# nvpro-samples/vk_gltf_renderer

Hardware: AMD Instinct MI355X
Metric: Msamples/s (and ms/frame @ fixed spp) 1080p & 4K, 1/2/4/8 MI355X (higher is better)
Workload: dtype f32

## Files before the change

### vk_gltf_renderer_amd/csrc/device/mi_pt_api.hip

```cpp
#include <hip/hip_runtime.h>

#include <algorithm>
#include <chrono>
#include <cstdlib>
#include <cmath>
#include <cstdio>
#include <cstring>
#include <memory>
#include <string>
#include <vector>

#include "mi_pt.h"
#include "bvh_refit.h"
#include "material_patch.h"
#include "pt_build.h"
#include "pt_bvh.h"
#include "pt_deform.h"
#include "pt_kernels.h"

namespace {

thread_local std::string g_lastError;

int fail(int code, const std::string& msg)
// ... 17 lines not shown
  size_t count = 0;
  hipError_t alloc(size_t n)
  {
    release();
    count = n;
    if(n == 0)
      return hipSuccess;
    return hipMalloc(reinterpret_cast<void**>(&ptr), n * sizeof(T));
  }
  hipError_t upload(const T* src, size_t n)
  {
    hipError_t e = alloc(n);
    if(e != hipSuccess || n == 0)
      return e;
    return hipMemcpy(ptr, src, n * sizeof(T), hipMemcpyHostToDevice);
  }
  void release()
  {
    if(ptr)
      (void)hipFree(ptr);
    ptr   = nullptr;
    count = 0;
  }
  ~DevBuf() { release(); }
};

enum TimedKernel { TK_GENERATE, TK_TRACE, TK_SORT, TK_SHADE, TK_SHADOW, TK_ACCUM, TK_PRIMARY, TK_SHADE_FIRST, TK_COUNT };

}

struct RunSwitches
{
  int    packetInterval = 1;
  int    sortMode       = 2;
  bool   noPacket       = false;
  bool   stateBySlot    = false;
  bool   traceSpans     = false;
  int    overlapUpTo    = 32;
  int    overlapMinTris = 200000;
  bool   noPlanes       = false;
  bool   noOpaqueTris   = false;
  bool   noQuads        = false;
  bool   shadowFarFirst = true;
  int    reinsert       = 16;
  int    reinsertUpdate = 0;
  int    reinsertRounds = 4;
  float  splitFactor    = 4.0f;
  int    splitMaxDepth  = 8;
  float  splitMinShare  = 0.1f;
  bool   collapseGreedy = false;
  bool   collapseBad    = false;
  bool   hostCollapse   = false;
  bool   coreTex        = true;
  int    maxItersDiag   = 0;
  int    failBuildAt    = 0;
  bool   candPoolSet    = false;
  size_t candPool       = 0;
  void   read()
  {
    auto flag = [](const char* n) { const char* e = getenv(n); return e != nullptr; };
    auto num  = [](const char* n, int d) { const char* e = getenv(n); return e ? atoi(e) : d; };
    packetInterval = num("MI_PT_PACKET_INTERVAL", 1);
    sortMode       = num("MI_PT_SORT", 2);
    noPacket       = flag("MI_PT_NO_PACKET");
    stateBySlot    = flag("MI_PT_STATE_BY_SLOT");
    traceSpans     = flag("MI_PT_TRACE_SPANS");
    overlapUpTo    = num("MI_PT_OVERLAP", 32);
    overlapMinTris = num("MI_PT_OVERLAP_MIN_TRIS", 200000);
    noPlanes       = flag("MI_PT_DIAG_NO_PLANES");
    noOpaqueTris   = flag("MI_PT_DIAG_NO_OPAQUE_TRIS");
    noQuads        = flag("MI_PT_DIAG_NO_QUADS");
    shadowFarFirst = num("MI_PT_SHADOW_FAR_FIRST", 1) != 0;
    reinsert       = std::max(0, num("MI_PT_REINSERT", 16));
    reinsertUpdate = std::max(0, num("MI_PT_REINSERT_UPDATE", 0));
    reinsertRounds = std::max(1, num("MI_PT_REINSERT_ROUNDS", 4));
    if(const char* e = getenv("MI_PT_SPLIT"))
      splitFactor = std::max(0.0f, float(atof(e)));
    if(const char* e = getenv("MI_PT_SPLIT_MIN_SHARE"))
      splitMinShare = std::max(0.0f, float(atof(e)));
    splitMaxDepth  = std::min(std::max(0, num("MI_PT_SPLIT_DEPTH", 8)), 10);
    if(const char* e = getenv("MI_PT_COLLAPSE"))
    {
      collapseGreedy = strcmp(e, "greedy") == 0;
      collapseBad    = !collapseGreedy && strcmp(e, "sah") != 0;
    }
    hostCollapse   = flag("MI_PT_HOST_COLLAPSE");
    maxItersDiag   = num("MI_PT_DIAG_MAX_ITERS", 0);
    coreTex        = num("MI_PT_CORE_TEX", 1) != 0;
    failBuildAt    = num("MI_PT_DIAG_FAIL_BUILD", 0);
    if(const char* e = getenv("MI_PT_DIAG_CAND_POOL"))
    {
      candPoolSet = true;
      candPool    = size_t(strtoull(e, nullptr, 10));
    }
  }
};

struct MiPt
{
  int device = 0;
  int numCUs = 256;
  RunSwitches sw;
  int accelBuilds = 0;
  int               frameQueueDepth = 1;
  int               pendingFrames   = 0;
  MiPathtraceParams pendingFirst{};
  void*             pendingStream   = nullptr;
  DevBuf<MiGltfShadeMaterial> materials;
  DevBuf<MiGltfTextureInfo>   texInfos;
  DevBuf<pt::DevTexRef>       texRefs;
  DevBuf<pt::DevCoreTex>      coreTex;
  DevBuf<MiGltfRenderNode>    nodes;
  DevBuf<pt::DevPrim>         prims;
  DevBuf<MiGltfLight>         lights;
  DevBuf<pt::DevTexture>      textures;
  DevBuf<uchar4>              texels;
  DevBuf<uint4>               texQuads;
  DevBuf<uint8_t>             geometry;
  DevBuf<uint8_t>             instFlags;
  DevBuf<float>               srgbLut;
  DevBuf<float4>              envPixels;
  DevBuf<MiEnvAccel>          envAccel;
  DevBuf<pt::DevAlphaTri>     alphaTris;
  DevBuf<pt::DevShadeTri>     shadeTris;
  float4*                     bvhNodes  = nullptr;
  uint4*                      bvh8Nodes = nullptr;
  DevBuf<float>               bvh8Planes;
  pt::DevTri*                 bvhTris   = nullptr;
  bool                        wide      = true;
  pt::DevScene                scene{};
  bool                        hasAlpha = false, hasAlphaTest = false, hasVolumeScatter = false, simpleMaterials = true, hasTransmissive = false;
  static constexpr int        FC_RING = 32;
  DevBuf<pt::DevScene>        sceneDev;
  bool                        sceneDevDirty = true;
  DevBuf<pt::FrameConsts>     fcRing;
  DevBuf<pt::SkyPrecomp>      skyPre;
  MiSkyPhysicalParameters     skyPreFor{};
  bool                        skyPreValid = false;
  pt::FrameConsts*            fcHost = nullptr;
  hipEvent_t                  fcDone[FC_RING] = {};
  unsigned                    fcCursor = 0;
// ... 1845 lines not shown
  }
  c.fc.skyPre    = pt->skyPre.ptr;
  c.fc.pc        = *params;
  c.fc.width     = pt->width;
  c.fc.height    = pt->height;
  c.fc.tileSize  = pt->tileSize;
  c.fc.tileShift = 0;
  while((1 << c.fc.tileShift) < pt->tileSize)
    ++c.fc.tileShift;
  c.fc.numSlots  = pt->numSlots;
  c.fc.numFrames = numFrames;
  pt::divideMagic(uint32_t(std::max(numFrames, 2)), c.fc.framesMagic, c.fc.framesShift);
  c.fc.slotLayout = numFrames % 64 == 0 ? 1 : 0;
  c.fc.stateInQueue = (!pt->sw.stateBySlot && !(pt->frameInfo.flags & MI_SCENE_INFINITE_PLANE_SHADOW_CATCHER)) ? 1 : 0;
  const bool guides = (params->flags & MI_PT_USE_OPTIX_DENOISER) != 0;
  if(int rc = ensureOptionalPathArrays(pt, c.fc.stateInQueue == 0, params->numSamples > 1, guides, (pt->frameInfo.flags & MI_SCENE_INFINITE_PLANE_SHADOW_CATCHER) != 0))
    return rc;
  c.paths        = pt->paths;
  {
    const bool stateBySlot = c.fc.stateInQueue == 0, multiSample = params->numSamples > 1;
    if(!(stateBySlot || multiSample))
      c.paths.misc = nullptr;
    if(!stateBySlot)
      c.paths.throughput = nullptr;
    if(!multiSample)
      c.paths.pixelSum = nullptr;
  }
  pt->accumFrames   = float(params->totalSamples) / float(params->numSamples) + float(numFrames);
  if(guides && (params->totalSamples == 0 || pt->momentFrames == pt->accumFrames - float(numFrames)))
    pt->momentFrames = pt->accumFrames;
  else if(!guides || params->totalSamples == 0)
    pt->momentFrames = 0.0f;
  if(!guides)
  {
    c.paths.guideAlbedo = nullptr;
    c.paths.guideNormal = nullptr;
  }
  c.queues           = pt->queues;
  if(!(pt->frameInfo.flags & MI_SCENE_INFINITE_PLANE_SHADOW_CATCHER))
    c.queues.shadow.aux2 = nullptr;
  c.ownedTiles       = pt->ownedTiles.ptr;
  c.stats            = pt->stats.ptr;
  c.stream           = stream;
  c.persistentBlocks = unsigned(pt->numCUs) * 8u;
  c.hasAlpha         = pt->hasAlpha;
  c.hasAlphaClosest  = c.hasAlpha && pt->hasAlphaTest;
  c.visualization    = pt->frameInfo.visualization > MI_VIZ_RENDERED && pt->frameInfo.visualization < MI_VIZ_COUNT;
  if(pt->frameInfo.visualization == MI_VIZ_OPACITY_MICROMAP)
    c.hasAlphaClosest = false;
  c.hasTransmissive  = pt->hasTransmissive;
  c.simpleMaterials  = pt->simpleMaterials;
  c.wide             = pt->wide;
  c.collectCounters  = pt->collectCounters;
  {
    c.sortMode = pt->sw.sortMode;
  }
  if(pt->sceneDevDirty)
  {
    HIP_TRY(hipDeviceSynchronize());
    HIP_TRY(pt->sceneDev.upload(&pt->scene, 1));
    pt->sceneDevDirty = false;
  }
  if(!pt->fcHost)
  {
    HIP_TRY(hipHostMalloc(reinterpret_cast<void**>(&pt->fcHost), sizeof(pt::FrameConsts) * MiPt::FC_RING, hipHostMallocDefault));
    HIP_TRY(pt->fcRing.alloc(MiPt::FC_RING));
    for(hipEvent_t& e : pt->fcDone)
      HIP_TRY(hipEventCreateWithFlags(&e, hipEventDisableTiming));
  }
  const unsigned fcSlot = pt->fcCursor++ % unsigned(MiPt::FC_RING);
  if(pt->fcCursor > unsigned(MiPt::FC_RING))
    HIP_TRY(hipEventSynchronize(pt->fcDone[fcSlot]));
  pt->fcHost[fcSlot] = c.fc;
  HIP_TRY(hipMemcpyAsync(pt->fcRing.ptr + fcSlot, pt->fcHost + fcSlot, sizeof(pt::FrameConsts), hipMemcpyHostToDevice, stream));
  c.sceneDev = pt->sceneDev.ptr;
  c.fcDev    = pt->fcRing.ptr + fcSlot;

  auto timedOn = [&](hipStream_t on, int kind, auto&& launch) {
    if(pt->timingEnabled)
    {
      hipEvent_t a = getEvent(pt, pt->evCursor), b = getEvent(pt, pt->evCursor);
      (void)hipEventRecord(a, on);
      launch();
      (void)hipEventRecord(b, on);
      pt->pendingSpans.push_back({kind, a, b});
    }
    else
      launch();
  };
  auto timed = [&](int kind, auto&& launch) { timedOn(stream, kind, launch); };
  hipEvent_t frameA = nullptr, frameB = nullptr;
  if(pt->timingEnabled)
  {
    frameA = getEvent(pt, pt->evCursor);
    frameB = getEvent(pt, pt->evCursor);
    (void)hipEventRecord(frameA, stream);
  }
  int iterations = 0, traceLaunches = 0, shadeLaunches = 0, shadowLaunches = 0;
  const bool usePacket = !pt->sw.noPacket;
  const bool debugSpans = pt->sw.traceSpans;
  bool overlap = pt->sw.overlapUpTo > 0 && ((numFrames <= pt->sw.overlapUpTo && pt->scene.numTris >= pt->sw.overlapMinTris) || pt->hasVolumeScatter)
                 && c.fc.stateInQueue != 0 && !debugSpans;
  if(overlap && !pt->sideStream)
    overlap = hipStreamCreateWithFlags(&pt->sideStream, hipStreamNonBlocking) == hipSuccess && hipEventCreateWithFlags(&pt->evShaded, hipEventDisableTiming) == hipSuccess
              && hipEventCreateWithFlags(&pt->evShadowed, hipEventDisableTiming) == hipSuccess;
  pt::LaunchCtx cSide = c;
// ... 618 lines not shown
```

### vk_gltf_renderer_amd/csrc/device/pt_kernels.h

```cpp
#pragma once
#include <hip/hip_runtime.h>

#include "pt_scene.h"
#include "pt_temporal.h"

namespace pt {

struct LaunchCtx
{
  DevScene        scene;
  FrameConsts     fc;
  const DevScene*    sceneDev;
  const FrameConsts* fcDev;
  PathSoA         paths;
  Queues          queues;
  const uint32_t* ownedTiles;
  StatCounters*   stats;
  hipStream_t     stream;
  unsigned        persistentBlocks;
  bool            hasAlpha;
  bool            hasAlphaClosest;
  bool            hasTransmissive;
  bool            simpleMaterials;
  bool            wide;
  bool            collectCounters;
  int             sortMode;
  bool            visualization;
};

void launchBuildShadeRecords(const DevScene& scene, uint32_t numTris, DevShadeTri* out, hipStream_t s);
void launchBuildAlphaRecords(const DevScene& scene, uint32_t numTris, DevAlphaTri* out, hipStream_t s);
void launchPatchMaterials(const DevScene& scene, const uint8_t* instFlags, const uint8_t* dirty, DevTri* tris, DevAlphaTri* alphaTris, DevShadeTri* shadeTris,
                          uint32_t numTris, hipStream_t s);
void dumpTraceProfile();
void launchBvh8Planes(const uint4* nodes, uint32_t numNodes, float* planes, hipStream_t s);
void launchTextureQuads(const uchar4* texels, uint4* quads, uint32_t offset, int width, int height, int wrapS, int wrapT, hipStream_t s);
void launchResetCounters(const Queues& Q, hipStream_t s);
void launchSkyPrecomp(const MiSkyPhysicalParameters& sky, SkyPrecomp* out, hipStream_t stream);
void launchGenerate(const LaunchCtx& c, int sampleIndex);
void launchTraceClosest(const LaunchCtx& c, int cur);
void launchTracePrimary(const LaunchCtx& c, int sampleIndex);
void launchShade(const LaunchCtx& c, int cur, bool first);
void launchTraceShadow(const LaunchCtx& c, int nxt);
void launchFlushSurvivors(const LaunchCtx& c, int cur);
void launchFinishSample(const LaunchCtx& c, int sampleIndex, float4* accum, float* depth, float4* albedo, float4* normal);
void launchSelection(const LaunchCtx& c, uint32_t* selection);

void launchAtrous(const float4* in, float4* out, const float4* albedo, const float4* normal, int width, int height, int step, float sigmaColor,
                  float sigmaNormal, float sigmaAlbedo, hipStream_t s);

const float4* launchSvgf(const float4* color, const float4* albedo, const float4* normal, const float* depth, float4* bufA, float4* bufB, int width, int height,
                         int iterations, float frames, float sigmaLuminance, float sigmaNormal, float sigmaDepth, hipStream_t s);

const float4* launchSvgfFilter(float4* in, float4* other, const float4* color, const float4* albedo, const float4* normal, const float* depth, int width,
                               int height, int iterations, float sigmaLuminance, float sigmaNormal, float sigmaDepth, hipStream_t s);

void launchMotionVectors(const float4* firstHit, const uint4* firstHitTri, const VertexMotionPrim* vmPrims, int numPrims, const uint32_t* ownedTiles,
                         uint32_t numSlots, int tileShift, int width, int height, const MiGltfRenderNode* nodes, float* prevObjectToWorld, int numNodes,
                         const float* viewProj, const float* prevMVP, float4* motion, hipStream_t s);
void launchSnapshotTransforms(const MiGltfRenderNode* nodes, float* prevObjectToWorld, int numNodes, hipStream_t s);
void launchSnapshotPositions(const VertexMotionPrim* vmPrims, const uint32_t* ids, uint32_t numIds, uint32_t maxVertexCount, hipStream_t s);
void launchSvgfReproject(const float4* color, const float4* albedo, const float4* normal, const float* depth, const float4* motion, const TemporalHistory& in,
                         const TemporalHistory& out, float4* illum, int width, int height, const TemporalConsts& tc, bool haveHistory, hipStream_t s);

void launchTonemap(const float4* in, uint32_t* outRgba8, int width, int height, const MiTonemapperData& tm, uint32_t* histogram, float* autoState,
                   float dtSeconds, hipStream_t s);

}
```

### vk_gltf_renderer_amd/csrc/device/pt_kernels.hip

```cpp
#include <hip/hip_runtime.h>
#include <hip/hip_fp16.h>

#ifndef MI_PT_EXACT_FP
#define PT_FAST_SHADING_MATH 1
#endif
#include "pt_kernels.h"
#include "pt_shading.h"
#include "pt_bvh.h"
#include "pt_bvh8.h"
#include "pt_packet.h"
#include "pt_feed.h"
#include "pt_visualize.h"

namespace pt {

namespace {

constexpr int TRACE_BLOCK = 1024;
#ifndef NODE_CACHE_EXTRA
#define NODE_CACHE_EXTRA 0
#endif
constexpr int NODE_CACHE  = 712 + NODE_CACHE_EXTRA;
constexpr int NODE_CACHE_ALPHA = 504 + NODE_CACHE_EXTRA;
constexpr int SEL_BLOCK   = 256;
// ... 1298 lines not shown
        const uint32_t child = groupPopChild(G, octinv);
        if(G.bits >> 8)
          st2.push(G);
        uint32_t tBase, tMask;
        bvh8Visit(sc, r, bestT, octinv, child, G, tBase, tMask, nullptr, 0u);
        while(leafPending(tMask))
        {
          const int k = int(leafPop(tMask, 0u));
          testTri(int(tBase) + k);
        }
      }
    }
    else
    {
      LaneStack st;
      int       stackOverflow[BVH_STACK_PRIV];
      st.lds = s_stack; st.tid = int(threadIdx.x); st.stride = SEL_BLOCK; st.sp = 0; st.priv = stackOverflow;
      bvhWalk(sc, r, bestT, st, [&](int triIndex, float) -> float {
        testTri(triIndex);
        return bestT;
      });
    }
  }
  selection[size_t(py) * size_t(fc.width) + size_t(px)] = (bestRnode != 0xffffffffu) ? bestRnode + 1u : 0u;
}

template <bool COUNT, bool SIMPLE, bool FIRST>
__global__ void __launch_bounds__(SHADE_BLOCK, SIMPLE ? SHADE_SIMPLE_WAVES : 1) k_shade(const DevScene* __restrict__ scp, const FrameConsts* __restrict__ fcp, PathSoA P, Queues Q, int cur, int sortMode, StatCounters* stats)
{
  constexpr bool VIZ = false;
#include "pt_shade_body.h"
}
template <bool SIMPLE, bool FIRST>
__global__ void __launch_bounds__(SHADE_BLOCK, SIMPLE ? SHADE_SIMPLE_WAVES : 1) k_shade_viz(const DevScene* __restrict__ scp, const FrameConsts* __restrict__ fcp, PathSoA P, Queues Q, int cur, int sortMode, StatCounters* stats)
{
  constexpr bool COUNT = false, VIZ = true;
#include "pt_shade_body.h"
}

template <int MODE>
struct ShadowCfg
{
  static constexpr int BLOCK = MODE == 2 ? 256 : TRACE_BLOCK;
  static constexpr int CACHE = MODE == 2 ? 320 : (MODE == 1 ? NODE_CACHE_ALPHA : (MODE == 3 ? NODE_CACHE_ALPHA - 104 : NODE_CACHE));
};

PT_DEV void shadowDeposit(const PathSoA& P, const Queues& Q, int nxt, uint32_t slot, uint32_t qpos, bool catcherRay, f3 contrib, f3 total, bool occ,
                          float catcherDarken)
{
  if(!catcherRay)
  {
    if(!occ)
    {
      float4* const target = (slot & SHADOW_TARGET_QUEUE) ? &Q.active[nxt].rad[slot & ~SHADOW_TARGET_QUEUE] : &P.radiance[slot];
      float4        rad    = *target;
      rad.x += contrib.x * total.x;
      rad.y += contrib.y * total.y;
      rad.z += contrib.z * total.z;
      *target = rad;
    }
    return;
  }
  const float4 a2  = Q.shadow.aux2[qpos];
  const f3     sf  = occ ? mk3(0.0f) : total;
  float4       rad = P.radiance[slot];
  if(sf.x == 1.0f && sf.y == 1.0f && sf.z == 1.0f)
  {
    rad.x += a2.x; rad.y += a2.y; rad.z += a2.z;
    const uint32_t posNext = __float_as_uint(a2.w);
    if(posNext != 0xffffffffu)
      Q.active[nxt].slot[posNext] = QUEUE_DEAD;
  }
  else
  {
    f3 r3 = mk3(rad.x, rad.y, rad.z);
    r3 += contrib * sf;
    r3 -= contrib * (mk3(1.0f) - sf) * catcherDarken;
    rad.x = r3.x; rad.y = r3.y; rad.z = r3.z;
  }
  P.radiance[slot] = rad;
}

template <bool WIDE, int MODE, bool COUNT>
__global__ void __launch_bounds__(ShadowCfg<MODE>::BLOCK, TRACE_MIN_WAVES) k_trace_shadow(DevScene sc, const DevScene* __restrict__ scp, PathSoA P, Queues Q, int nxt, float catcherDarken, StatCounters* stats, int overflowOnly)
{
  constexpr int  SBLOCK    = ShadowCfg<MODE>::BLOCK;
  constexpr bool HAS_ALPHA = MODE >= 1, HAS_TRANS = MODE == 2, REC = MODE == 3;
  constexpr bool DEFER = MODE == 1 || MODE == 3;
  static_assert(!REC || WIDE, "the recording walk exists for the 8-wide BVH only");
  __shared__ int      s_stack[BVH_STACK_LDS * SBLOCK];
  __shared__ uint32_t s_prefix[NSUB + 1];
  __shared__ uint4    s_nodes[WIDE ? ShadowCfg<MODE>::CACHE * 5 : 1];
  __shared__ uint32_t s_items[(WIDE && !HAS_TRANS) ? SBLOCK : 1];
  __shared__ uint4    s_alpha[(WIDE && DEFER) ? SBLOCK : 1];
  __shared__ uint32_t s_head[REC ? SBLOCK : 1], s_ovf[REC ? SBLOCK : 1];
  __shared__ uint8_t  s_octLut[(WIDE && MI_PT_OCT_LUT) ? OCT_LUT_BYTES : 1];
  queuePrefix(&Q.counters[(nxt ? QC_PAIR1 : QC_PAIR0) + 1], s_prefix);
  const RayQueue in = Q.shadow;
  const bool     subset = MODE == 2 && overflowOnly != 0;
  uint32_t* const heads = &Q.counters[subset ? QC_HEADS_OVERFLOW : QC_HEADS_SHADOW];
  WaveFeed feed;
  feedInit(feed, subset ? Q.counters[QC_OVERFLOW] : s_prefix[NSUB]);
  if(!feedBlockHasWork(feed))
    return;
  if(WIDE && MI_PT_OCT_LUT)
    fillOctLut(s_octLut);
  const uint32_t cachedNodes = WIDE ? fillNodeCache(sc, s_nodes, uint32_t(ShadowCfg<MODE>::CACHE)) : 0u;
  LaneStack  st;
  LaneStack2 st2;
  int        stackOverflow[WIDE ? 2 * BVH8_STACK_PRIV : BVH_STACK_PRIV];
  st.lds = s_stack;  st.tid = int(threadIdx.x);  st.stride = SBLOCK;  st.sp = 0;  st.priv = stackOverflow;
  st2.lds = s_stack; st2.tid = int(threadIdx.x); st2.stride = SBLOCK; st2.sp = 0;
  st2.privBase = reinterpret_cast<uint32_t*>(stackOverflow); st2.privBits = reinterpret_cast<uint32_t*>(stackOverflow) + (WIDE ? BVH8_STACK_PRIV : 0);
  bool      active = false;
  uint32_t  slot   = 0;
  RaySetup  r{};
  int       node = BVH_EMPTY;
  NodeGroup G{0, 0};
  uint32_t  octinv = 0;
  float     tMax  = 0.0f;
  int       phase = 0;
  unsigned  nTrans = 0;
  bool      occluded = false;
  uint32_t  seed0 = 0;
  f3        contrib = mk3(0.0f);
  float    bT = 0.0f, bU = 0.0f, bV = 0.0f, lastT = -1.0f, prevHitT = 0.0f;
  uint32_t bRnode = 0, bPrim = 0, lastRnode = 0, lastPrim = 0;
  int      bTri = 0;
  bool     found = false, haveLast = false, isInside = false;
  f3       total = mk3(1.0f);
  unsigned nodes = 0, tris = 0, rays = 0;
  bool     pValid = false;
  uint32_t pSlot = QUEUE_DEAD, pQPos = 0, qpos = 0;
  float4   pO = make_float4(0, 0, 0, 0), pD = make_float4(0, 0, 0, 0), pC = make_float4(0, 0, 0, 0);
  bool     catcherRay = false;
  uint32_t pBase = 0, pMask = 0, qBase = 0, qMask = 0;
  uint32_t aCount   = 0;
  bool     aPending = false;
  bool     toOverflow = false;
#ifdef TRACE_PROFILE
  unsigned long long sp[16] = {0, 0, 0, 0, 0, 0, 0, 0, 0, 0, 0, 0, 0, 0, 0, 0};
  const unsigned long long spStart = PROF_T();
#define SPROF_ADD(i, t0) sp[i] += PROF_T() - (t0)
#define SPROF_CNT(i, n) sp[i] += (unsigned long long)(n)
#else
#define SPROF_ADD(i, t0) (void)(t0)
#define SPROF_CNT(i, n) (void)0
#endif
  uint4*   waveAlpha = s_alpha + ((WIDE && DEFER) ? (threadIdx.x & ~63u) : 0u);
  CandRec  rec{Q.candPool, Q.candNext, &Q.counters[QC_CAND_POOL], Q.candCap, s_head + (REC ? (threadIdx.x & ~63u) : 0u), s_ovf + (REC ? (threadIdx.x & ~63u) : 0u), 0u, 0u};
  (void)rec;

  auto deposit = [&](bool occ) { shadowDeposit(P, Q, nxt, slot, qpos, catcherRay, contrib, total, occ, catcherDarken); };

  constexpr unsigned SHADOW_CANDS = 8;
  float    cT[HAS_TRANS ? SHADOW_CANDS : 1], cU[HAS_TRANS ? SHADOW_CANDS : 1], cV[HAS_TRANS ? SHADOW_CANDS : 1];
  uint32_t cR[HAS_TRANS ? SHADOW_CANDS : 1], cP[HAS_TRANS ? SHADOW_CANDS : 1];
  int      cI[HAS_TRANS ? SHADOW_CANDS : 1];
  auto processCandidate = [&](float t, int tri, uint32_t rnode, uint32_t prim, float u, float v) {
    f3    bary    = mk3(1.0f - u - v, u, v);
    float opacity = getOpacityFast(sc, tri, bary);
    if(candidateRand(seed0, int(rnode), int(prim)) < opacity)
    {
      float segment = fmaxf(0.0f, t - prevHitT);
      f3    curT    = getShadowTransmission(*scp, int(rnode), int(prim), bary, segment, r.dir, isInside);
      prevHitT      = t;
      total *= curT;
      if(maxComp(total) <= MIN_TRANSMISSION)
        occluded = true;
    }
  };

  auto restartWalk = [&]() {
    if(WIDE)
    {
      G      = rootGroup(octinv);
      st2.sp = 0;
      pMask = qMask = 0u;
    }
    else
    {
      st.sp = 0;
      node  = sc.bvhRoot;
    }
  };
  auto testTriLoaded = [&](const DevTri& T, int triIndex) {
    if(COUNT) ++tris;
    const uint32_t flags = __float_as_uint(T.c.w);
    TriHit         h;
    const bool consider = !HAS_TRANS || phase == 0 || ((flags & INST_TRANSMISSIVE) && !(flags & INST_FORCE_OPAQUE));
    if(!(consider && intersectTri(xyz(T.a), xyz(T.b), xyz(T.c), r.org, r.dir, h) && h.t > 0.0f && h.t < tMax))
      return;
    const uint32_t rnode = __float_as_uint(T.a.w), prim = __float_as_uint(T.b.w);
    if(!HAS_TRANS || phase == 0)
    {
      if(!HAS_ALPHA || (flags & INST_FORCE_OPAQUE))
        occluded = true;
      else if(HAS_TRANS && (flags & INST_TRANSMISSIVE))
      {
        if(nTrans < SHADOW_CANDS)
        {
          cT[nTrans] = h.t; cI[nTrans] = triIndex; cR[nTrans] = rnode; cP[nTrans] = prim; cU[nTrans] = h.u; cV[nTrans] = h.v;
        }
        ++nTrans;
      }
      else
      {
        float opacity = getOpacityFast(sc, triIndex, mk3(1.0f - h.u - h.v, h.u, h.v));
        if(candidateRand(seed0, int(rnode), int(prim)) < opacity)
          occluded = true;
      }
    }
    else
    {
      const bool afterLast  = !haveLast || h.t > lastT || (h.t == lastT && (rnode > lastRnode || (rnode == lastRnode && prim > lastPrim)));
      const bool beforeBest = !found || h.t < bT || (h.t == bT && (rnode < bRnode || (rnode == bRnode && prim < bPrim)));
      if(afterLast && beforeBest)
      {
        found = true; bT = h.t; bTri = triIndex; bRnode = rnode; bPrim = prim; bU = h.u; bV = h.v;
      }
    }
  };

  auto testTri = [&](int triIndex) { testTriLoaded(sc.tris[triIndex], triIndex); };

  for(;;)
  {
    const unsigned long long tOuter = PROF_T();
    SPROF_CNT(8, 1);
    SPROF_CNT(9, 64 - __popcll(__ballot(active)));
    if(!active && pValid)
    {
      pValid = false;
      if(pSlot != QUEUE_DEAD)
      {
        slot     = pSlot;
        qpos     = pQPos;
        r        = makeRaySetup(xyz(pO), xyz(pD));
        tMax     = pO.w;
        isInside = (__float_as_uint(pD.w) & 1u) != 0u;
        catcherRay = (__float_as_uint(pD.w) & 2u) != 0u;
        contrib  = xyz(pC);
        seed0    = __float_as_uint(pC.w);
        phase    = 0;
        nTrans   = 0;
        occluded = false;
        total    = mk3(1.0f);
        haveLast = false;
        found    = false;
        prevHitT = 0.0f;
        octinv   = rayOctInv(r.idir) ^ (MODE == 2 ? 0u : sc.shadowOctFlip);
        restartWalk();
        active = true;
        if(REC)
        {
          s_head[threadIdx.x] = CAND_NIL;
          s_ovf[threadIdx.x]  = 0u;
        }
        if(COUNT) ++rays;
        if(sc.bvhRoot == BVH_EMPTY)
        {
          if(HAS_TRANS)
            deposit(false);
          else
            reinterpret_cast<uint32_t*>(&Q.shadow.org[qpos])[3] = CAND_NIL;
          active = false;
        }
      }
    }
    if(!feed.exhausted)
    {
      uint32_t flat = feedTake(feed, !pValid, heads);
      if(flat != 0xffffffffu)
      {
        const uint32_t pPos = subset ? Q.overflow[flat] : queuePos(Q.subCap, s_prefix, flat);
        pQPos  = pPos;
        pSlot  = in.slot[pPos];
        pO     = in.org[pPos];
        pD     = in.dir[pPos];
        pC     = in.aux[pPos];
        pValid = true;
      }
    }
    const bool moreWork = !feed.exhausted || __ballot(pValid) != 0ull;
    SPROF_ADD(0, tOuter);
    if(__ballot(active) == 0ull)
    {
      if(!moreWork)
        break;
      continue;
    }
    for(;;)
    {
      bool walkDone = false;
      const unsigned long long tInner = PROF_T();
      SPROF_CNT(10, 1);
      SPROF_CNT(11, __popcll(__ballot(active)));
      if(WIDE)
      {
        bool visited = false;
        if(active && !leafPending(qMask) && !(DEFER && occluded))
        {
          const float walkTmax = (HAS_TRANS && phase == 1 && found) ? bT : tMax;
          if((G.bits >> 8) == 0u && st2.sp > 0)
            G = st2.pop();
          if(G.bits >> 8)
          {
            const uint32_t child = groupPopChild(G, octinv);
            if(G.bits >> 8)
              st2.push(G);
            uint32_t tBase, tMask;
            bvh8Visit(sc, r, walkTmax, octinv, child, G, tBase, tMask, s_nodes, cachedNodes, s_octLut);
            if(COUNT) ++nodes;
            visited = true;
            if(leafPending(tMask))
            {
              if(!leafPending(pMask)) { pBase = tBase; pMask = tMask; }
              else                    { qBase = tBase; qMask = tMask; }
            }
          }
        }
// ... 73 lines not shown
        }
        if(node < 0 && node != BVH_EMPTY)
        {
          testTri(~node);
          node = bvhPop(st);
        }
        walkDone = occluded || node == BVH_EMPTY;
      }
      const unsigned long long tFin = PROF_T();
      if(active)
      {
        if(walkDone)
        {
          bool finished = true;
          if(HAS_TRANS && !occluded && phase == 0 && nTrans > 0 && nTrans <= SHADOW_CANDS)
          {
            for(unsigned k = 0; k < nTrans && !occluded; ++k)
            {
              int best = -1;
              for(unsigned j = 0; j < nTrans; ++j)
              {
                const bool afterLast  = !haveLast || cT[j] > lastT || (cT[j] == lastT && (cR[j] > lastRnode || (cR[j] == lastRnode && cP[j] > lastPrim)));
                const bool beforeBest = best < 0 || cT[j] < cT[best] || (cT[j] == cT[best] && (cR[j] < cR[best] || (cR[j] == cR[best] && cP[j] < cP[best])));
                if(afterLast && beforeBest)
                  best = int(j);
              }
              if(best < 0)
                break;
              haveLast = true; lastT = cT[best]; lastRnode = cR[best]; lastPrim = cP[best];
              processCandidate(cT[best], cI[best], cR[best], cP[best], cU[best], cV[best]);
            }
            nTrans = 0;
          }
          if(HAS_TRANS && !occluded && !(phase == 1 && !found))
          {
            if(phase == 1)
            {
              haveLast = true; lastT = bT; lastRnode = bRnode; lastPrim = bPrim;
              processCandidate(bT, bTri, bRnode, bPrim, bU, bV);
              --nTrans;
            }
            if(!occluded && nTrans > 0)
            {
              phase = 1;
              found = false;
              restartWalk();
              finished = false;
            }
          }
          if(finished)
          {
            if(HAS_TRANS)
              deposit(occluded);
            else
            {
              uint32_t code = occluded ? SHADOW_OCCLUDED : CAND_NIL;
              if(REC && !occluded)
              {
                code       = s_head[threadIdx.x];
                toOverflow = s_ovf[threadIdx.x] != 0u;
              }
              if(toOverflow)
                reinterpret_cast<uint32_t*>(&Q.shadow.dir[qpos])[3] |= SHADOW_DIR_OVERFLOW;
              else
                reinterpret_cast<uint32_t*>(&Q.shadow.org[qpos])[3] = code;
            }
            active = false;
          }
        }
      }
      if(REC)
      {
        const unsigned long long mO = __ballot(toOverflow);
        if(mO != 0ull)
        {
          const int first = __ffsll((long long)mO) - 1;
          uint32_t  base  = 0u;
          if(int(laneId()) == first)
            base = atomicAdd(&Q.counters[QC_OVERFLOW], uint32_t(__popcll(mO)));
          base = uint32_t(__builtin_amdgcn_readlane(int(base), first));
          if(toOverflow)
            Q.overflow[base + laneCountBelow(mO)] = qpos;
        }
        toOverflow = false;
      }
      SPROF_ADD(4, tFin);
      const unsigned long long act = __ballot(active);
      if(act == 0ull || (moreWork && __popcll(act) <= 64 - REFILL_IDLE_LANES))
        break;
    }
  }
#ifdef TRACE_PROFILE
  if(laneId() == 0 && WIDE && DEFER)
  {
    sp[5] = PROF_T() - spStart;
    sp[6] = 1;
    for(int i = 0; i < 16; ++i)
      atomicAdd(&g_shadowProf[i], sp[i]);
  }
#endif
#undef SPROF_ADD
#undef SPROF_CNT
  if(COUNT)
  {
    atomicAdd(&stats->shadowRays, (unsigned long long)rays);
    atomicAdd(&stats->nodesShadow, (unsigned long long)nodes);
    atomicAdd(&stats->trisShadow, (unsigned long long)tris);
  }
}

PT_DEV void resolveChain(const DevScene& sc, const PathSoA& P, const Queues& Q, int nxt, uint32_t qpos, uint32_t slot, float4 d4, float4 c4, uint32_t code, bool catcherRay,
                         float catcherDarken)
{
  f3             total    = mk3(1.0f);
  bool           occluded = false;
  const f3       dir      = xyz(d4);
  const uint32_t seed0    = __float_as_uint(c4.w);
  bool           isInside = (__float_as_uint(d4.w) & 1u) != 0u, haveLast = false;
  float          lastT = -1.0f, prevHitT = 0.0f;
  uint32_t       lastRnode = 0u, lastPrim = 0u;
  for(;;)
  {
    uint32_t best = CAND_NIL, bRnode = 0u, bPrim = 0u;
    bool     bIds = false;
    float4   bC   = make_float4(0, 0, 0, 0);
    for(uint32_t k = code; k != CAND_NIL; k = Q.candNext[k])
    {
      const float4   c   = Q.candPool[k];
      const uint32_t tri = __float_as_uint(c.w);
      const bool     tieLast = haveLast && c.x == lastT, tieBest = best != CAND_NIL && c.x == bC.x;
      uint32_t       rnode = 0u, prim = 0u;
      if(tieLast || tieBest)
      {
        rnode = __float_as_uint(gat(sc.tris, tri).a.w);
        prim  = __float_as_uint(gat(sc.tris, tri).b.w);
      }
      const bool afterLast  = !haveLast || c.x > lastT || (tieLast && (rnode > lastRnode || (rnode == lastRnode && prim > lastPrim)));
      bool       beforeBest = best == CAND_NIL || c.x < bC.x;
      if(tieBest)
      {
        if(!bIds)
        {
          const uint32_t bt = __float_as_uint(bC.w);
          bRnode = __float_as_uint(gat(sc.tris, bt).a.w);
          bPrim  = __float_as_uint(gat(sc.tris, bt).b.w);
          bIds   = true;
        }
        beforeBest = rnode < bRnode || (rnode == bRnode && prim < bPrim);
      }
      if(afterLast && beforeBest)
      {
        best = k; bC = c; bRnode = rnode; bPrim = prim; bIds = tieLast || tieBest;
      }
    }
    if(best == CAND_NIL)
      break;
    const uint32_t tri = __float_as_uint(bC.w);
    const uint32_t rnode = __float_as_uint(gat(sc.tris, tri).a.w), prim = __float_as_uint(gat(sc.tris, tri).b.w);
    haveLast = true; lastT = bC.x; lastRnode = rnode; lastPrim = prim;
    const f3    bary    = mk3(1.0f - bC.y - bC.z, bC.y, bC.z);
    const bool  passes  = (__float_as_uint(gat(sc.tris, tri).c.w) & INST_ALPHA_PASSES) != 0u;
    if(passes || candidateRand(seed0, int(rnode), int(prim)) < getOpacityFast(sc, int(tri), bary))
    {
      const float segment = fmaxf(0.0f, bC.x - prevHitT);
      const f3    curT    = getShadowTransmissionTri(sc, int(rnode), int(prim), int(tri), bary, segment, dir, isInside);
      prevHitT            = bC.x;
      total *= curT;
      if(maxComp(total) <= MIN_TRANSMISSION)
      {
        occluded = true;
        break;
      }
    }
  }
  if(occluded && !catcherRay)
    return;
  shadowDeposit(P, Q, nxt, slot, qpos, catcherRay, xyz(c4), total, occluded, catcherDarken);
}

template <bool REC>
__global__ void __launch_bounds__(256) k_shadow_resolve(const DevScene* __restrict__ scp, PathSoA P, Queues Q, int nxt, float catcherDarken)
{
  __shared__ uint32_t s_prefix[NSUB + 1];
#ifndef RESOLVE_INLINE_CHAINS
  constexpr bool LIST = REC;
#else
  constexpr bool LIST = false;
#endif
  __shared__ uint32_t s_chain[LIST ? 512 : 1];
  __shared__ uint32_t s_chainCount;
  if(threadIdx.x == 0)
    s_chainCount = 0;
  queuePrefix(&Q.counters[(nxt ? QC_PAIR1 : QC_PAIR0) + 1], s_prefix);
  const uint32_t  count = s_prefix[NSUB];
  const DevScene& sc    = uniformConst(*scp);
  auto workOff = [&](bool all) {
    __syncthreads();
    const uint32_t n = s_chainCount;
    if(n == 0u || (!all && n < 256u))
      return;
    const uint32_t take = min(n, 256u), base = n - take;
    uint32_t       qpos = 0;
    if(threadIdx.x < take)
      qpos = s_chain[base + threadIdx.x];
    __syncthreads();
    if(threadIdx.x == 0)
      s_chainCount = base;
    if(threadIdx.x < take)
    {
      const float4 d4 = Q.shadow.dir[qpos];
      resolveChain(sc, P, Q, nxt, qpos, Q.shadow.slot[qpos], d4, Q.shadow.aux[qpos], reinterpret_cast<const uint32_t*>(&Q.shadow.org[qpos])[3], (__float_as_uint(d4.w) & 2u) != 0u,
                   catcherDarken);
    }
    __syncthreads();
  };
  const uint32_t rounds = (count + gridDim.x * blockDim.x - 1u) / (gridDim.x * blockDim.x);
  for(uint32_t it = 0; it < rounds; ++it)
  {
    const uint32_t i = it * gridDim.x * blockDim.x + blockIdx.x * blockDim.x + threadIdx.x;
    if(i < count)
    {
      const uint32_t qpos = queuePos(Q.subCap, s_prefix, i);
      const uint32_t slot = Q.shadow.slot[qpos];
      const float4   d4   = slot != QUEUE_DEAD ? Q.shadow.dir[qpos] : make_float4(0, 0, 0, 0);
      if(slot != QUEUE_DEAD && !(REC && (__float_as_uint(d4.w) & SHADOW_DIR_OVERFLOW)))
      {
        const uint32_t code       = reinterpret_cast<const uint32_t*>(&Q.shadow.org[qpos])[3];
        const bool     catcherRay = (__float_as_uint(d4.w) & 2u) != 0u;
        const bool     occluded   = code == SHADOW_OCCLUDED;
        if(!occluded || catcherRay)
        {
          if(REC && !occluded && code != CAND_NIL)
          {
            if(LIST)
              s_chain[atomicAdd(&s_chainCount, 1u)] = qpos;
            else
              resolveChain(sc, P, Q, nxt, qpos, slot, d4, Q.shadow.aux[qpos], code, catcherRay, catcherDarken);
          }
          else
            shadowDeposit(P, Q, nxt, slot, qpos, catcherRay, xyz(Q.shadow.aux[qpos]), mk3(1.0f), occluded, catcherDarken);
        }
      }
    }
    if(LIST)
      workOff(false);
  }
  if(LIST)
  {
    workOff(true);
    workOff(true);
  }
}

__global__ void __launch_bounds__(256) k_flush_survivors(PathSoA P, Queues Q, int cur)
{
  __shared__ uint32_t s_prefix[NSUB + 1];
  queuePrefix(&Q.counters[cur ? QC_PAIR1 : QC_PAIR0], s_prefix);
  const uint32_t count = s_prefix[NSUB];
  for(uint32_t i = blockIdx.x * blockDim.x + threadIdx.x; i < count; i += gridDim.x * blockDim.x)
  {
    const uint32_t qpos = queuePos(Q.subCap, s_prefix, i);
    const uint32_t slot = Q.active[cur].slot[qpos];
    if(slot == QUEUE_DEAD)
      continue;
    P.radiance[slot] = Q.active[cur].rad[qpos];
    if(P.misc)
      P.misc[slot] = Q.active[cur].misc[qpos];
  }
}

#ifndef FINISH_AHEAD
#define FINISH_AHEAD 4
#endif
__global__ void __launch_bounds__(256) k_finish_sample(FrameConsts fc, const DevScene* __restrict__ scp, const FrameConsts* __restrict__ fcp, PathSoA P,
                                                       const uint32_t* ownedTiles, int sampleIndex, float4* accum, float* depth, float4* albedoOut,
                                                       float4* normalOut)
{
  const uint32_t pslot = blockIdx.x * blockDim.x + threadIdx.x;
  int            px, py;
  if(pslot >= uint32_t(fc.numSlots) || !slotToPixel(fc, ownedTiles, pslot, px, py))
    return;
  const size_t idx      = size_t(py) * size_t(fc.width) + size_t(px);
  const bool   lastSample = sampleIndex + 1 >= fc.pc.numSamples;
// ... 213 lines not shown
{
  const uint32_t n = uint32_t(width) * uint32_t(height);
  hipLaunchKernelGGL(k_texture_quads, dim3((n + 255u) / 256u), dim3(256), 0, s, reinterpret_cast<const uint32_t*>(texels), quads, offset, width, height, wrapS, wrapT);
}
void launchResetCounters(const Queues& Q, hipStream_t s)
{
  hipLaunchKernelGGL(k_reset_counters, dim3(1), dim3(64), 0, s, Q.counters);
}
__global__ void k_sky_precomp(MiSkyPhysicalParameters sky, SkyPrecomp* out)
{
  if(blockIdx.x == 0 && threadIdx.x == 0)
    *out = makeSkyPrecomp(sky);
}
void launchSkyPrecomp(const MiSkyPhysicalParameters& sky, SkyPrecomp* out, hipStream_t stream)
{
  hipLaunchKernelGGL(k_sky_precomp, dim3(1), dim3(64), 0, stream, sky, out);
}

void launchGenerate(const LaunchCtx& c, int sampleIndex)
{
  unsigned grid = (unsigned(c.fc.numSlots) * unsigned(c.fc.numFrames) + 255u) / 256u;
  hipLaunchKernelGGL(k_generate, dim3(grid), dim3(256), 0, c.stream, c.scene, c.fc, c.paths, c.queues, c.ownedTiles, sampleIndex,
                     c.collectCounters ? c.stats : nullptr);
}
namespace {
template <bool WIDE>
void launchTraceClosestT(const LaunchCtx& c, int cur)
{
  dim3 grid(c.persistentBlocks * 256u / TRACE_BLOCK), block(TRACE_BLOCK);
  if(c.hasAlphaClosest)
  {
    if(c.collectCounters)
      hipLaunchKernelGGL((k_trace_closest<WIDE, true, true>), grid, block, 0, c.stream, c.scene, c.paths, c.queues, cur, c.stats);
    else
      hipLaunchKernelGGL((k_trace_closest<WIDE, true, false>), grid, block, 0, c.stream, c.scene, c.paths, c.queues, cur, c.stats);
  }
  else
  {
    if(c.collectCounters)
      hipLaunchKernelGGL((k_trace_closest<WIDE, false, true>), grid, block, 0, c.stream, c.scene, c.paths, c.queues, cur, c.stats);
    else
      hipLaunchKernelGGL((k_trace_closest<WIDE, false, false>), grid, block, 0, c.stream, c.scene, c.paths, c.queues, cur, c.stats);
  }
}
template <bool WIDE>
void launchTraceShadowT(const LaunchCtx& c, int nxt)
{
  const float darken = c.fc.frameInfo.shadowCatcherDarkenAmount;
  const bool  record = WIDE && c.hasAlpha && c.hasTransmissive && c.queues.candPool != nullptr;
  const int   mode   = !c.hasAlpha ? 0 : (c.hasTransmissive ? (record ? 3 : 2) : 1);
  const unsigned bs  = mode == 2 ? unsigned(ShadowCfg<2>::BLOCK) : unsigned(ShadowCfg<0>::BLOCK);
  dim3 grid(c.persistentBlocks * 256u / bs), block(bs);
#define MI_LAUNCH_SHADOW(M, C, OVF) \
  hipLaunchKernelGGL((k_trace_shadow<WIDE, M, C>), grid, block, 0, c.stream, c.scene, c.sceneDev, c.paths, c.queues, nxt, darken, c.stats, OVF)
  const dim3 rgrid(c.persistentBlocks), rblock(256);
  if(mode == 0)      { if(c.collectCounters) MI_LAUNCH_SHADOW(0, true, 0); else MI_LAUNCH_SHADOW(0, false, 0); }
  else if(mode == 1) { if(c.collectCounters) MI_LAUNCH_SHADOW(1, true, 0); else MI_LAUNCH_SHADOW(1, false, 0); }
  else if(mode == 2) { if(c.collectCounters) MI_LAUNCH_SHADOW(2, true, 0); else MI_LAUNCH_SHADOW(2, false, 0); }
  else
  {
    if constexpr(WIDE)
    {
      if(c.collectCounters) MI_LAUNCH_SHADOW(3, true, 0); else MI_LAUNCH_SHADOW(3, false, 0);
    }
  }
  if(mode == 3)
  {
    hipLaunchKernelGGL(k_shadow_resolve<true>, rgrid, rblock, 0, c.stream, c.sceneDev, c.paths, c.queues, nxt, darken);
    if constexpr(WIDE)
    {
      grid  = dim3(c.persistentBlocks * 256u / unsigned(ShadowCfg<2>::BLOCK));
      block = dim3(unsigned(ShadowCfg<2>::BLOCK));
      if(c.collectCounters) MI_LAUNCH_SHADOW(2, true, 1); else MI_LAUNCH_SHADOW(2, false, 1);
    }
  }
  else if(mode != 2)
    hipLaunchKernelGGL(k_shadow_resolve<false>, rgrid, rblock, 0, c.stream, c.sceneDev, c.paths, c.queues, nxt, darken);
#undef MI_LAUNCH_SHADOW
}
}
void launchTracePrimary(const LaunchCtx& c, int sampleIndex)
{
  const uint32_t batchSlots = uint32_t(c.fc.numSlots) * uint32_t(c.fc.numFrames);
  dim3           grid(batchSlots / 256u), block(256);
  const bool interval = c.fc.slotLayout == 1 && c.scene.packetInterval != 0 && c.scene.bvh8Planes != nullptr;
#define MI_LAUNCH_PRIMARY(A, C)                                                                                                                   \
  do                                                                                                                                              \
  {                                                                                                                                               \
    if(interval)                                                                                                                                  \
      hipLaunchKernelGGL((k_trace_primary<A, C, true>), grid, block, 0, c.stream, c.scene, c.fc, c.sceneDev, c.fcDev, c.paths, c.queues, c.ownedTiles, sampleIndex, batchSlots, c.stats);  \
    else                                                                                                                                          \
      hipLaunchKernelGGL((k_trace_primary<A, C, false>), grid, block, 0, c.stream, c.scene, c.fc, c.sceneDev, c.fcDev, c.paths, c.queues, c.ownedTiles, sampleIndex, batchSlots, c.stats); \
  } while(0)
  if(c.hasAlphaClosest)
  {
    if(c.collectCounters) MI_LAUNCH_PRIMARY(true, true); else MI_LAUNCH_PRIMARY(true, false);
  }
  else
  {
    if(c.collectCounters) MI_LAUNCH_PRIMARY(false, true); else MI_LAUNCH_PRIMARY(false, false);
  }
#undef MI_LAUNCH_PRIMARY
}
void launchTraceClosest(const LaunchCtx& c, int cur)
{
  if(c.wide)
    launchTraceClosestT<true>(c, cur);
  else
    launchTraceClosestT<false>(c, cur);
}
void launchShade(const LaunchCtx& c, int cur, bool first)
{
  dim3 grid(c.persistentBlocks), block(SHADE_BLOCK);
  if(c.visualization)
  {
#define MI_LAUNCH_SHADE_VIZ(S, F) \
  hipLaunchKernelGGL((k_shade_viz<S, F>), grid, block, 0, c.stream, c.sceneDev, c.fcDev, c.paths, c.queues, cur, (S ? 0 : c.sortMode), c.stats)
    if(c.simpleMaterials)
    {
      if(first) MI_LAUNCH_SHADE_VIZ(true, true); else MI_LAUNCH_SHADE_VIZ(true, false);
    }
    else
    {
      if(first) MI_LAUNCH_SHADE_VIZ(false, true); else MI_LAUNCH_SHADE_VIZ(false, false);
    }
#undef MI_LAUNCH_SHADE_VIZ
    return;
  }
#define MI_LAUNCH_SHADE(C, S, F) \
  hipLaunchKernelGGL((k_shade<C, S, F>), grid, block, 0, c.stream, c.sceneDev, c.fcDev, c.paths, c.queues, cur, (S ? 0 : c.sortMode), c.stats)
// ... 39 lines not shown
```

### vk_gltf_renderer_amd/csrc/device/pt_scene.h

```cpp
#pragma once
#include <hip/hip_runtime.h>
#include <stdint.h>

#include "mi_pt.h"
#include "pt_math.h"

namespace pt {

struct DevTexture
{
  uint32_t levelOffset[16];
  uint16_t width, height;
  uint8_t  numLevels;
  uint8_t  srgb;
  uint8_t  magFilter, minFilter, mipmapMode, wrapS, wrapT;
  uint8_t  _pad[5];
};

struct DevTexRef
{
  float    uv[6];
  uint32_t level0;
  uint16_t width, height;
  uint8_t  numLevels, srgb, magFilter, minFilter, mipmapMode, wrapS, wrapT, texCoord;
// ... 213 lines not shown
{
  PF_INSIDE     = 1u << 0,
  PF_NOT_SOLID  = 1u << 1,
  PF_ALIVE      = 1u << 2,
  PF_PLANE_HIT  = 1u << 3,
  PF_PRIMARY_MISS = 1u << 4,
  PF_DEPTH_SHIFT   = 8,
  PF_SCATTER_SHIFT = 16,
};
constexpr uint32_t RADW_NOT_SOLID    = 0x80000000u;
constexpr uint32_t RADW_PRIMARY_MISS = 0xffc00001u;

struct PathSoA
{
  float4*   radiance;
  float4*   firstHit;
  float4*   misc;
  float4*   throughput;
  uint4*    medium;
  float4*   pixelSum;
  float4*   guideAlbedo;
  float4*   guideNormal;
  uint4*    firstHitTri;
};

constexpr int      NSUB       = 16;
constexpr int      QCHUNK     = 256;
constexpr uint32_t QUEUE_DEAD = 0xffffffffu;
struct RayQueue
{
  uint32_t* slot;
  float4*   org;
  float4*   dir;
  float4*   aux;
  float4*   aux2;
  float4*   misc;
  float4*   rad;
};
constexpr uint32_t SHADOW_TARGET_QUEUE = 0x80000000u;
struct Queues
{
  RayQueue  active[2];
  RayQueue  shadow;
  uint32_t* counters;
  uint32_t  subCap;
  float4*   candPool;
  uint32_t* candNext;
  uint32_t* overflow;
  uint32_t  candCap;
};
constexpr uint32_t CAND_NIL        = 0xffffffffu;
constexpr uint32_t SHADOW_OCCLUDED = 0xfffffffeu;
constexpr uint32_t SHADOW_DIR_OVERFLOW = 4u;
enum : int
{
  QC_PAIR0        = 0,
  QC_PAIR1        = 32,
  QC_HEADS_TRACE  = 96,
  QC_HEADS_SHADOW = 128,
  QC_HEADS_OVERFLOW = 160,
  QC_CAND_POOL      = 192,
  QC_RESOLVE        = 224,
  QC_OVERFLOW       = 256,
  QC_COUNT          = 288
};

struct StatCounters
{
  unsigned long long cameraPaths, segments, shadowRays, nodesClosest, trisClosest, nodesShadow, trisShadow, textureTaps, surfaceHits, nodesPrimary, trisPrimary;
};

}
```

Before: 747.1.

## Deposit unoccluded shadow contributions in-walk via atomics, skipping resolve pass

For opaque and alpha shadow modes, the shadow trace kernel now adds unoccluded light contributions straight into the path radiance target with float atomics, instead of writing a code that a separate resolve kernel reads later. The resolve kernel is then skipped unless shadow-catcher rays exist, and in that case it only handles catcher rays. This removes a kernel launch and a pass over the shadow queue. In exchange it adds three atomic adds per lit ray, makes the summation order nondeterministic, and for the wide alpha mode loads the contribution late to save registers.

```diff
diff --git a/vk_gltf_renderer_amd/csrc/device/mi_pt_api.hip b/vk_gltf_renderer_amd/csrc/device/mi_pt_api.hip
--- a/vk_gltf_renderer_amd/csrc/device/mi_pt_api.hip
+++ b/vk_gltf_renderer_amd/csrc/device/mi_pt_api.hip
@@ -93,6 +93,7 @@
   bool   collapseBad    = false;
   bool   hostCollapse   = false;
   bool   coreTex        = true;
+  bool   shadowDeposit  = true;
   int    maxItersDiag   = 0;
   int    failBuildAt    = 0;
   bool   candPoolSet    = false;
@@ -128,6 +129,7 @@
     hostCollapse   = flag("MI_PT_HOST_COLLAPSE");
     maxItersDiag   = num("MI_PT_DIAG_MAX_ITERS", 0);
     coreTex        = num("MI_PT_CORE_TEX", 1) != 0;
+    shadowDeposit  = num("MI_PT_SHADOW_DEPOSIT", 1) != 0;
     failBuildAt    = num("MI_PT_DIAG_FAIL_BUILD", 0);
     if(const char* e = getenv("MI_PT_DIAG_CAND_POOL"))
     {
@@ -2079,6 +2081,7 @@
   c.simpleMaterials  = pt->simpleMaterials;
   c.wide             = pt->wide;
   c.collectCounters  = pt->collectCounters;
+  c.shadowDeposit    = pt->sw.shadowDeposit;
   {
     c.sortMode = pt->sw.sortMode;
   }
diff --git a/vk_gltf_renderer_amd/csrc/device/pt_kernels.h b/vk_gltf_renderer_amd/csrc/device/pt_kernels.h
--- a/vk_gltf_renderer_amd/csrc/device/pt_kernels.h
+++ b/vk_gltf_renderer_amd/csrc/device/pt_kernels.h
@@ -24,6 +24,7 @@
   bool            simpleMaterials;
   bool            wide;
   bool            collectCounters;
+  bool            shadowDeposit;
   int             sortMode;
   bool            visualization;
 };
diff --git a/vk_gltf_renderer_amd/csrc/device/pt_kernels.hip b/vk_gltf_renderer_amd/csrc/device/pt_kernels.hip
--- a/vk_gltf_renderer_amd/csrc/device/pt_kernels.hip
+++ b/vk_gltf_renderer_amd/csrc/device/pt_kernels.hip
@@ -1374,7 +1374,7 @@
   {
     if(!occ)
     {
-      float4* const target = (slot & SHADOW_TARGET_QUEUE) ? &Q.active[nxt].rad[slot & ~SHADOW_TARGET_QUEUE] : &P.radiance[slot];
+      float4* const target = shadowTarget(P, Q, nxt, slot);
       float4        rad    = *target;
       rad.x += contrib.x * total.x;
       rad.y += contrib.y * total.y;
@@ -1404,11 +1404,14 @@
 }
 
 template <bool WIDE, int MODE, bool COUNT>
-__global__ void __launch_bounds__(ShadowCfg<MODE>::BLOCK, TRACE_MIN_WAVES) k_trace_shadow(DevScene sc, const DevScene* __restrict__ scp, PathSoA P, Queues Q, int nxt, float catcherDarken, StatCounters* stats, int overflowOnly)
+__global__ void __launch_bounds__(ShadowCfg<MODE>::BLOCK, TRACE_MIN_WAVES) k_trace_shadow(DevScene sc, const DevScene* __restrict__ scp, PathSoA P, Queues Q, int nxt, float catcherDarken, StatCounters* stats, int overflowOnly,
+                                                                                          int walkDeposit)
 {
   constexpr int  SBLOCK    = ShadowCfg<MODE>::BLOCK;
   constexpr bool HAS_ALPHA = MODE >= 1, HAS_TRANS = MODE == 2, REC = MODE == 3;
   constexpr bool DEFER = MODE == 1 || MODE == 3;
+  const bool inWalk = !HAS_TRANS && !REC && walkDeposit != 0;
+  constexpr bool LATE_CONTRIB = WIDE && MODE == 1;
   static_assert(!REC || WIDE, "the recording walk exists for the 8-wide BVH only");
   __shared__ int      s_stack[BVH_STACK_LDS * SBLOCK];
   __shared__ uint32_t s_prefix[NSUB + 1];
@@ -1453,13 +1456,15 @@
   f3       total = mk3(1.0f);
   unsigned nodes = 0, tris = 0, rays = 0;
   bool     pValid = false;
-  uint32_t pSlot = QUEUE_DEAD, pQPos = 0, qpos = 0;
+  uint32_t pSlot = QUEUE_DEAD, pQPos = 0;
+  uint32_t posOrTarget = 0;
   float4   pO = make_float4(0, 0, 0, 0), pD = make_float4(0, 0, 0, 0), pC = make_float4(0, 0, 0, 0);
   bool     catcherRay = false;
   uint32_t pBase = 0, pMask = 0, qBase = 0, qMask = 0;
   uint32_t aCount   = 0;
   bool     aPending = false;
   bool     toOverflow = false;
+  bool     lateContrib = false;
 #ifdef TRACE_PROFILE
   unsigned long long sp[16] = {0, 0, 0, 0, 0, 0, 0, 0, 0, 0, 0, 0, 0, 0, 0, 0};
   const unsigned long long spStart = PROF_T();
@@ -1473,7 +1478,7 @@
   CandRec  rec{Q.candPool, Q.candNext, &Q.counters[QC_CAND_POOL], Q.candCap, s_head + (REC ? (threadIdx.x & ~63u) : 0u), s_ovf + (REC ? (threadIdx.x & ~63u) : 0u), 0u, 0u};
   (void)rec;
 
-  auto deposit = [&](bool occ) { shadowDeposit(P, Q, nxt, slot, qpos, catcherRay, contrib, total, occ, catcherDarken); };
+  auto deposit = [&](bool occ) { shadowDeposit(P, Q, nxt, slot, posOrTarget, catcherRay, contrib, total, occ, catcherDarken); };
 
   constexpr unsigned SHADOW_CANDS = 8;
   float    cT[HAS_TRANS ? SHADOW_CANDS : 1], cU[HAS_TRANS ? SHADOW_CANDS : 1], cV[HAS_TRANS ? SHADOW_CANDS : 1];
@@ -1556,13 +1561,14 @@
       pValid = false;
       if(pSlot != QUEUE_DEAD)
       {
+        catcherRay = (__float_as_uint(pD.w) & 2u) != 0u;
         slot     = pSlot;
-        qpos     = pQPos;
+        posOrTarget     = (inWalk && !catcherRay) ? pSlot : pQPos;
         r        = makeRaySetup(xyz(pO), xyz(pD));
         tMax     = pO.w;
         isInside = (__float_as_uint(pD.w) & 1u) != 0u;
-        catcherRay = (__float_as_uint(pD.w) & 2u) != 0u;
-        contrib  = xyz(pC);
+        if(!LATE_CONTRIB)
+          contrib = xyz(pC);
         seed0    = __float_as_uint(pC.w);
         phase    = 0;
         nTrans   = 0;
@@ -1582,13 +1588,30 @@
         if(COUNT) ++rays;
         if(sc.bvhRoot == BVH_EMPTY)
         {
-          if(HAS_TRANS)
-            deposit(false);
+          if(!HAS_TRANS && inWalk && !catcherRay)
+          {
+            G    = NodeGroup{0, 0};
+            node = BVH_EMPTY;
+          }
           else
-            reinterpret_cast<uint32_t*>(&Q.shadow.org[qpos])[3] = CAND_NIL;
-          active = false;
+          {
+            if(HAS_TRANS)
+              deposit(false);
+            else
+              reinterpret_cast<uint32_t*>(&Q.shadow.org[posOrTarget])[3] = CAND_NIL;
+            active = false;
+          }
         }
-      }
+        lateContrib = LATE_CONTRIB && inWalk && active && !catcherRay;
+      }
+    }
+    if(lateContrib)
+    {
+      lateContrib = false;
+      const float* const a = reinterpret_cast<const float*>(&in.aux[pQPos]);
+      contrib.x = __hip_atomic_load(a + 0, __ATOMIC_RELAXED, __HIP_MEMORY_SCOPE_WAVEFRONT);
+      contrib.y = __hip_atomic_load(a + 1, __ATOMIC_RELAXED, __HIP_MEMORY_SCOPE_WAVEFRONT);
+      contrib.z = __hip_atomic_load(a + 2, __ATOMIC_RELAXED, __HIP_MEMORY_SCOPE_WAVEFRONT);
     }
     if(!feed.exhausted)
     {
@@ -1768,6 +1791,11 @@
           {
             if(HAS_TRANS)
               deposit(occluded);
+            else if(inWalk && !catcherRay)
+            {
+              if(!occluded)
+                shadowDepositAdd(shadowTarget(P, Q, nxt, posOrTarget), contrib);
+            }
             else
             {
               uint32_t code = occluded ? SHADOW_OCCLUDED : CAND_NIL;
@@ -1777,9 +1805,9 @@
                 toOverflow = s_ovf[threadIdx.x] != 0u;
               }
               if(toOverflow)
-                reinterpret_cast<uint32_t*>(&Q.shadow.dir[qpos])[3] |= SHADOW_DIR_OVERFLOW;
+                reinterpret_cast<uint32_t*>(&Q.shadow.dir[posOrTarget])[3] |= SHADOW_DIR_OVERFLOW;
               else
-                reinterpret_cast<uint32_t*>(&Q.shadow.org[qpos])[3] = code;
+                reinterpret_cast<uint32_t*>(&Q.shadow.org[posOrTarget])[3] = code;
             }
             active = false;
           }
@@ -1796,7 +1824,7 @@
             base = atomicAdd(&Q.counters[QC_OVERFLOW], uint32_t(__popcll(mO)));
           base = uint32_t(__builtin_amdgcn_readlane(int(base), first));
           if(toOverflow)
-            Q.overflow[base + laneCountBelow(mO)] = qpos;
+            Q.overflow[base + laneCountBelow(mO)] = posOrTarget;
         }
         toOverflow = false;
       }
@@ -1895,7 +1923,7 @@
 }
 
 template <bool REC>
-__global__ void __launch_bounds__(256) k_shadow_resolve(const DevScene* __restrict__ scp, PathSoA P, Queues Q, int nxt, float catcherDarken)
+__global__ void __launch_bounds__(256) k_shadow_resolve(const DevScene* __restrict__ scp, PathSoA P, Queues Q, int nxt, float catcherDarken, int catcherOnly)
 {
   __shared__ uint32_t s_prefix[NSUB + 1];
 #ifndef RESOLVE_INLINE_CHAINS
@@ -1904,7 +1932,7 @@
   constexpr bool LIST = false;
 #endif
   __shared__ uint32_t s_chain[LIST ? 512 : 1];
-  __shared__ uint32_t s_chainCount;
+  __shared__ uint32_t s_chainCount, s_chainSeen;
   if(threadIdx.x == 0)
     s_chainCount = 0;
   queuePrefix(&Q.counters[(nxt ? QC_PAIR1 : QC_PAIR0) + 1], s_prefix);
@@ -1912,7 +1940,10 @@
   const DevScene& sc    = uniformConst(*scp);
   auto workOff = [&](bool all) {
     __syncthreads();
-    const uint32_t n = s_chainCount;
+    if(threadIdx.x == 0)
+      s_chainSeen = s_chainCount;
+    __syncthreads();
+    const uint32_t n = s_chainSeen;
     if(n == 0u || (!all && n < 256u))
       return;
     const uint32_t take = min(n, 256u), base = n - take;
@@ -1944,7 +1975,7 @@
         const uint32_t code       = reinterpret_cast<const uint32_t*>(&Q.shadow.org[qpos])[3];
         const bool     catcherRay = (__float_as_uint(d4.w) & 2u) != 0u;
         const bool     occluded   = code == SHADOW_OCCLUDED;
-        if(!occluded || catcherRay)
+        if((!occluded || catcherRay) && (REC || catcherRay || catcherOnly == 0))
         {
           if(REC && !occluded && code != CAND_NIL)
           {
@@ -2264,7 +2295,9 @@
   const unsigned bs  = mode == 2 ? unsigned(ShadowCfg<2>::BLOCK) : unsigned(ShadowCfg<0>::BLOCK);
   dim3 grid(c.persistentBlocks * 256u / bs), block(bs);
 #define MI_LAUNCH_SHADOW(M, C, OVF) \
-  hipLaunchKernelGGL((k_trace_shadow<WIDE, M, C>), grid, block, 0, c.stream, c.scene, c.sceneDev, c.paths, c.queues, nxt, darken, c.stats, OVF)
+  hipLaunchKernelGGL((k_trace_shadow<WIDE, M, C>), grid, block, 0, c.stream, c.scene, c.sceneDev, c.paths, c.queues, nxt, darken, c.stats, OVF, deposit)
+  const int  deposit     = (c.shadowDeposit && (mode == 0 || mode == 1)) ? 1 : 0;
+  const bool catcherRays = (c.fc.frameInfo.flags & MI_SCENE_USE_INFINITE_PLANE) && (c.fc.frameInfo.flags & MI_SCENE_INFINITE_PLANE_SHADOW_CATCHER);
   const dim3 rgrid(c.persistentBlocks), rblock(256);
   if(mode == 0)      { if(c.collectCounters) MI_LAUNCH_SHADOW(0, true, 0); else MI_LAUNCH_SHADOW(0, false, 0); }
   else if(mode == 1) { if(c.collectCounters) MI_LAUNCH_SHADOW(1, true, 0); else MI_LAUNCH_SHADOW(1, false, 0); }
@@ -2278,7 +2311,7 @@
   }
   if(mode == 3)
   {
-    hipLaunchKernelGGL(k_shadow_resolve<true>, rgrid, rblock, 0, c.stream, c.sceneDev, c.paths, c.queues, nxt, darken);
+    hipLaunchKernelGGL(k_shadow_resolve<true>, rgrid, rblock, 0, c.stream, c.sceneDev, c.paths, c.queues, nxt, darken, 0);
     if constexpr(WIDE)
     {
       grid  = dim3(c.persistentBlocks * 256u / unsigned(ShadowCfg<2>::BLOCK));
@@ -2286,8 +2319,8 @@
       if(c.collectCounters) MI_LAUNCH_SHADOW(2, true, 1); else MI_LAUNCH_SHADOW(2, false, 1);
     }
   }
-  else if(mode != 2)
-    hipLaunchKernelGGL(k_shadow_resolve<false>, rgrid, rblock, 0, c.stream, c.sceneDev, c.paths, c.queues, nxt, darken);
+  else if(mode != 2 && (!deposit || catcherRays))
+    hipLaunchKernelGGL(k_shadow_resolve<false>, rgrid, rblock, 0, c.stream, c.sceneDev, c.paths, c.queues, nxt, darken, deposit);
 #undef MI_LAUNCH_SHADOW
 }
 }
diff --git a/vk_gltf_renderer_amd/csrc/device/pt_scene.h b/vk_gltf_renderer_amd/csrc/device/pt_scene.h
--- a/vk_gltf_renderer_amd/csrc/device/pt_scene.h
+++ b/vk_gltf_renderer_amd/csrc/device/pt_scene.h
@@ -289,6 +289,19 @@
 constexpr uint32_t CAND_NIL        = 0xffffffffu;
 constexpr uint32_t SHADOW_OCCLUDED = 0xfffffffeu;
 constexpr uint32_t SHADOW_DIR_OVERFLOW = 4u;
+#ifdef __HIPCC__
+PT_DEV void shadowDepositAdd(float4* target, f3 c)
+{
+  float* const p = reinterpret_cast<float*>(target);
+  (void)__hip_atomic_fetch_add(p + 0, c.x, __ATOMIC_RELAXED, __HIP_MEMORY_SCOPE_AGENT);
+  (void)__hip_atomic_fetch_add(p + 1, c.y, __ATOMIC_RELAXED, __HIP_MEMORY_SCOPE_AGENT);
+  (void)__hip_atomic_fetch_add(p + 2, c.z, __ATOMIC_RELAXED, __HIP_MEMORY_SCOPE_AGENT);
+}
+PT_DEV float4* shadowTarget(const PathSoA& P, const Queues& Q, int nxt, uint32_t slot)
+{
+  return (slot & SHADOW_TARGET_QUEUE) ? &Q.active[nxt].rad[slot & ~SHADOW_TARGET_QUEUE] : &P.radiance[slot];
+}
+#endif
 enum : int
 {
   QC_PAIR0        = 0,
```

Result: faster. 756.1, median of 6 (+1.2%).
